# wenxiaoshuai/Points-Matching

Measured on AMD Instinct MI355X. Metric: descriptor-pair distances/s (BF-L2 2-NN + ratio stage); RANSAC hypotheses/s in `ransac`, higher is better.
Workload: dtype f32

## Files before the change

### include/pm.h

```cpp
#ifndef PM_H_
#define PM_H_

#include <stddef.h>
#include <stdint.h>

#ifdef __cplusplus
extern "C" {
#endif

#define PM_VERSION_MAJOR 0
#define PM_VERSION_MINOR 1

typedef enum pm_status {
    PM_OK            =  0,
    PM_E_INVALID     = -1,
    PM_E_TOO_FEW     = -2,
    PM_E_NO_MODEL    = -3,
    PM_E_HIP         = -4,
    PM_E_NOMEM       = -5,
    PM_E_UNSUPPORTED = -6
} pm_status;

typedef struct pm_match {
    int32_t queryIdx;
// ... 7 lines not shown
int  pm_ctx_create(int device, pm_ctx** out);
int  pm_ctx_destroy(pm_ctx* ctx);
int  pm_ctx_set_stream(pm_ctx* ctx, void* hip_stream);
int  pm_ctx_synchronize(pm_ctx* ctx);
int  pm_device_alloc(pm_ctx* ctx, size_t bytes, void** d_out);
int  pm_device_free(pm_ctx* ctx, void* d_ptr);
int  pm_device_upload(pm_ctx* ctx, void* d_dst, const void* src, size_t bytes);
int  pm_device_download(pm_ctx* ctx, void* dst, const void* d_src, size_t bytes);
int  pm_ctx_timing_enable(pm_ctx* ctx, int enable);
int  pm_ctx_timing_reset(pm_ctx* ctx);
int  pm_ctx_timing_get(pm_ctx* ctx, const char* kernel, double* mean_ms, int* launches);
int  pm_ctx_knn_diag_enable(pm_ctx* ctx, int enable);
int  pm_ctx_knn_stats(pm_ctx* ctx, int* rescans, int* nonfinite);
int  pm_ctx_knn_route(pm_ctx* ctx, int* route);
int  pm_ctx_filter_fusion_status(pm_ctx* ctx, int* gave_up);
enum {
    PM_OPT_RANSAC_PATH    = 1,
    PM_OPT_SCORE_OPERANDS = 2,
    PM_OPT_HAMMING_ROUTE  = 3,
    PM_OPT_KNN_F16_WAVES  = 4,
    PM_OPT_KNN_STAGING    = 6,
    PM_OPT_KNN_WG_PER_CU  = 7,
    PM_OPT_FILTER_FUSION  = 5,
    PM_OPT_KNN_XCD_TILE   = 8,
    PM_OPT_KNN_GENERAL_F16 = 9,
    PM_OPT_KNN_SEEDED     = 10,
    PM_OPT_KNN_U8_GROUP   = 11,
    PM_OPT_KNN_RING       = 12,
    PM_OPT_KNN_U8_REFINE  = 13,
    PM_OPT_KNN_RING_PROLOGUE = 14,
// ... 418 lines not shown
```

### points_matching_amd/api.py

```python
import ctypes as C
import os

import numpy as np

_HERE = os.path.dirname(os.path.abspath(__file__))
LIB_PATH = os.environ.get("PM_LIB_PATH") or os.path.join(_HERE, "libpm_hip.so")

MATCH_DTYPE = np.dtype([("queryIdx", "<i4"), ("trainIdx", "<i4"), ("imgIdx", "<i4"),
                        ("distance", "<f4")])
PM_MAX_K = 16
PM_KNN_FORCE_EXACT = 1
PM_KNN_FORCE_F32 = 2
PM_KNN_HINT_INTEGER = 4
PM_KNN_HINT_U8 = 8
PM_KNN_HINT_UNIT_NORM = 16
PM_CROSS_RATIO_FWD = 1
PM_CROSS_RATIO_REV = 2
PM_GUIDE_F_SAMPSON = 0
PM_GUIDE_F_SYM = 1
PM_GUIDE_H = 2
PM_ERR_SAMPSON = 0
PM_ERR_SYM_EPIPOLAR = 1
PM_ERR_REPROJ = 2
PM_AFFINE_FULL = 0
PM_AFFINE_PARTIAL = 1
PM_OK, PM_E_INVALID, PM_E_TOO_FEW, PM_E_NO_MODEL, PM_E_HIP, PM_E_NOMEM, PM_E_UNSUPPORTED = \
    0, -1, -2, -3, -4, -5, -6

EXPORTS = [
    "pm_ctx_create", "pm_ctx_destroy", "pm_ctx_set_stream", "pm_ctx_synchronize",
    "pm_ctx_timing_enable", "pm_ctx_timing_reset", "pm_ctx_timing_get", "pm_ctx_knn_diag_enable", "pm_ctx_knn_stats", "pm_ctx_knn_route",
    "pm_ctx_filter_fusion_status",
    "pm_last_error",
    "pm_status_string", "pm_version",
    "pm_bf_knn_l2_f32", "pm_bf_knn_l2_f32_dev", "pm_bf_knn_hamming_u8", "pm_bf_knn_hamming_u8_dev",
    "pm_filter_midpoint", "pm_filter_ratio", "pm_match_indices", "pm_gather_points",
    "pm_format_match_list",
    "pm_filter_ratio_gather_dev", "pm_filter_midpoint_gather_dev", "pm_concat_points_dev",
    "pm_ransac_fundamental", "pm_ransac_score_dev", "pm_ransac_score_devn", "pm_ransac_model_from_hyp",
    "pm_ransac_model_from_key_dev", "pm_ransac_run_dev", "pm_ransac_shard_parts_dev", "pm_ransac_finish_parts_dev",
    "pm_ctx_set_option", "pm_ctx_get_option", "pm_bf_knn_l2_ratio_dev",
    "pm_flann_build", "pm_flann_destroy", "pm_flann_knn_l2_f32", "pm_flann_knn_l2_f32_dev", "pm_flann_export",
    "pm_mgpu_create", "pm_mgpu_destroy", "pm_mgpu_size", "pm_mgpu_ctx", "pm_mgpu_ransac_fundamental", "pm_mgpu_match_ransac",
    "pm_mgpu_lane_ctx", "pm_mgpu_set_lanes", "pm_mgpu_set_train", "pm_mgpu_set_train_dev", "pm_mgpu_submit_dev", "pm_mgpu_collect",
    "pm_mgpu_allgather_latency", "pm_mgpu_batch_run", "pm_mgpu_batch_set_option",
    "pm_batch_create", "pm_batch_destroy", "pm_batch_run", "pm_batch_set_option", "pm_batch_set_desc_type", "pm_batch_set_host_threads",
    "pm_bf_knn_l2_u8", "pm_bf_knn_l2_u8_dev", "pm_bf_knn_l2_u8_ratio_dev", "pm_host_register", "pm_host_unregister",
# ... 331 lines not shown
    def ransac_finish_parts_dev(self, view, thresh_px, drecs_ptr, n_records, dkey_ptr, dF_ptr, dmask_ptr, mask_len,
                                dninl_ptr, dntotal_ptr=0, kind=PM_ERR_SAMPSON):
        prm = RansacParams(0, 0, 0, thresh_px, kind)
        _check(lib().pm_ransac_finish_parts_dev(self._h, C.byref(view), C.byref(prm), C.c_void_p(drecs_ptr), n_records,
                                                C.c_void_p(dkey_ptr or 0), C.c_void_p(dF_ptr or 0), C.c_void_p(dmask_ptr),
                                                mask_len, C.c_void_p(dninl_ptr or 0), C.c_void_p(dntotal_ptr or 0)))

    def knn_diag_enable(self, on=True):
        _check(lib().pm_ctx_knn_diag_enable(self._h, int(on)))

    def filter_fusion_gave_up(self):
        g = C.c_int()
        _check(lib().pm_ctx_filter_fusion_status(self._h, C.byref(g)))
        return g.value

    def knn_stats(self):
        r, nf = C.c_int(), C.c_int()
        _check(lib().pm_ctx_knn_stats(self._h, C.byref(r), C.byref(nf)))
        rt = C.c_int()
        _check(lib().pm_ctx_knn_route(self._h, C.byref(rt)))
        return {"rescans": r.value, "nonfinite": nf.value, "route": rt.value}

    def filter_ratio_gather_dev(self, dknn_ptr, nq, k, ratio, dkp1_ptr, dkp2_ptr, dgood_ptr, dxy1_ptr,
                                dxy2_ptr, dn_ptr):
        _check(lib().pm_filter_ratio_gather_dev(self._h, C.c_void_p(dknn_ptr), nq, k, C.c_float(ratio),
                                                C.c_void_p(dkp1_ptr), C.c_void_p(dkp2_ptr),
                                                C.c_void_p(dgood_ptr), C.c_void_p(dxy1_ptr),
                                                C.c_void_p(dxy2_ptr), C.c_void_p(dn_ptr)))

    def filter_cross_gather_dev(self, dfwd_ptr, nq, kf, drev_ptr, nt, kr, cross_flags, ratio, dkp1_ptr, dkp2_ptr, dgood_ptr,
# ... 936 lines not shown
```

### points_matching_amd/csrc/pm_capi.cpp

```cpp
#include <cfloat>
#include <cmath>

#include "pm_common.hpp"

namespace pm {

static thread_local char g_err[512] = "";

void set_error(const char* fmt, ...)
{
    va_list ap;
    va_start(ap, fmt);
    vsnprintf(g_err, sizeof g_err, fmt, ap);
    va_end(ap);
}

int arena_reserve(pm_ctx* ctx, size_t bytes)
{
    if (bytes <= ctx->arena_cap) return PM_OK;
    PM_HIP_CHECK(hipStreamSynchronize(ctx->stream));
    if (ctx->arena) PM_HIP_CHECK(hipFree(ctx->arena));
    ctx->arena = nullptr;
    ctx->arena_cap = 0;
    size_t cap = align_up(bytes + bytes / 4, size_t(1) << 20);
// ... 161 lines not shown
    *out = c;
    return PM_OK;
}

int pm_ctx_destroy(pm_ctx* ctx)
{
    if (!ctx) return PM_OK;
    (void)hipSetDevice(ctx->device);
    (void)hipStreamSynchronize(ctx->stream);
    drain_timers(ctx);
    for (hipEvent_t e : ctx->event_pool) (void)hipEventDestroy(e);
    if (ctx->arena) (void)hipFree(ctx->arena);
    if (ctx->knn_stats) (void)hipFree(ctx->knn_stats);
    if (ctx->fg_counts) (void)hipFree(ctx->fg_counts);
    if (ctx->sync_words) (void)hipFree(ctx->sync_words);
    if (ctx->kf_tile) (void)hipFree(ctx->kf_tile);
    if (ctx->widen) (void)hipFree(ctx->widen);
    if (ctx->feat) (void)hipFree(ctx->feat);
    if (ctx->pinned) (void)hipHostFree(ctx->pinned);
    if (ctx->own_stream) (void)hipStreamDestroy(ctx->own_stream);
    delete ctx;
    return PM_OK;
}

int pm_ctx_set_stream(pm_ctx* ctx, void* hip_stream)
{
    PM_REQUIRE(ctx != nullptr, PM_E_INVALID, "ctx is null");
    PM_HIP_CHECK(hipStreamSynchronize(ctx->stream));
    ctx->stream = hip_stream ? static_cast<hipStream_t>(hip_stream) : ctx->own_stream;
    return PM_OK;
// ... 102 lines not shown

int pm_ctx_knn_diag_enable(pm_ctx* ctx, int enable)
{
    PM_REQUIRE(ctx != nullptr, PM_E_INVALID, "ctx is null");
    ctx->knn_diag = enable != 0;
    return PM_OK;
}

int pm_ctx_filter_fusion_status(pm_ctx* ctx, int* gave_up)
{
    PM_REQUIRE(ctx != nullptr && gave_up != nullptr, PM_E_INVALID, "null argument");
    unsigned w = 0;
    PM_HIP_CHECK(hipStreamSynchronize(ctx->stream));
    PM_HIP_CHECK(hipMemcpy(&w, reinterpret_cast<const char*>(ctx->knn_stats) + 48, sizeof w, hipMemcpyDeviceToHost));
    *gave_up = (ctx->kf_epoch != 0u && w == ctx->kf_epoch) ? 1 : 0;
    return PM_OK;
}

int pm_ctx_knn_stats(pm_ctx* ctx, int* rescans, int* nonfinite)
{
    PM_REQUIRE(ctx != nullptr, PM_E_INVALID, "ctx is null");
    unsigned h[2] = {0, 0};
    PM_HIP_CHECK(hipStreamSynchronize(ctx->stream));
    PM_HIP_CHECK(hipMemcpy(h, ctx->knn_diag_words, sizeof h, hipMemcpyDeviceToHost));
    if (rescans) *rescans = static_cast<int>(h[0]);
    if (nonfinite) *nonfinite = static_cast<int>(h[1]);
    return PM_OK;
}

int pm_ctx_knn_route(pm_ctx* ctx, int* route)
// ... 206 lines not shown
```

### points_matching_amd/csrc/pm_common.hpp

```cpp
#pragma once
#include <hip/hip_runtime.h>

#include <cstdarg>
#include <cstdint>
#include <cstdio>
#include <cstring>
#include <map>
#include <string>
#include <vector>

#include "pm.h"
#include "stage_layout.hpp"

namespace pm {

void set_error(const char* fmt, ...);

#define PM_HIP_CHECK(expr)                                                              \
    do {                                                                                \
        hipError_t e_ = (expr);                                                         \
        if (e_ != hipSuccess) {                                                         \
            ::pm::set_error("%s failed: %s (%s:%d)", #expr, hipGetErrorString(e_),      \
                            __FILE__, __LINE__);                                        \
            return PM_E_HIP;                                                            \
// ... 38 lines not shown
    size_t pinned_cap = 0;
    bool timing = false;
    std::map<std::string, pm::KernelTimer> timers;
    std::vector<hipEvent_t> event_pool;
    int n_cu = 256;
    unsigned long long* knn_stats = nullptr;
    unsigned* knn_diag_words = nullptr;
    unsigned knn_epoch = 0;
    bool knn_diag = false;
    unsigned* fg_counts = nullptr;
    unsigned fg_epoch = 0;
    unsigned long long* kf_tile = nullptr;
    int kf_cap = 0;
    unsigned kf_epoch = 0;
    int* sync_words = nullptr;
    int opts[PM_OPT_COUNT_] = {};
    float* widen = nullptr;
    size_t widen_cap = 0;
    char* feat = nullptr;
    size_t feat_cap = 0;
    size_t feat_counter_off = 0;
    int feat_noct = 0;
    int feat_w[16] = {}, feat_h[16] = {};
    size_t feat_off[16] = {};
};

namespace pm {

int arena_reserve(pm_ctx* ctx, size_t bytes);
void arena_reset(pm_ctx* ctx);
// ... 83 lines not shown
```

### points_matching_amd/csrc/ransac_a_fused.hip

```cpp
#include "affine_core.hpp"
#include "ransac_fused_kernels.hpp"

namespace pm_ransac {
namespace {

using namespace pm_affine;

constexpr int RA_SYNC_WORD = 12;

template <int MODEL>
struct AModel {
    static constexpr int MIN_PTS = Traits<MODEL>::MIN_PTS;
    static constexpr bool SHARD_OUT = false;
    static constexpr int OUT_WORDS = 6;
    static constexpr bool CANDIDATES = false;

    template <typename DIAG>
    static __device__ __forceinline__ bool solve(const pm_points_view& v, const int* __restrict__ offs, int n, uint64_t seed,
                                                 uint64_t h, double (&A)[9])
    {
        int idx[MIN_PTS];
        sample<MODEL>(seed, h, n, idx);
        double x1[MIN_PTS], y1[MIN_PTS], x2[MIN_PTS], y2[MIN_PTS];
#pragma unroll
// ... 20 lines not shown
    }

    static __device__ __forceinline__ void inlier_x2(const float (&a)[9], f32x2 x, f32x2 y, f32x2 xp, f32x2 yp, float thr2,
                                                     bool& ia, bool& ib)
    {
        inlier_a32_x2(a, x, y, xp, yp, thr2, ia, ib);
    }
};

}

int ransac_a_enqueue(pm_ctx* ctx, int model, const pm_points_view& v, const pm_ransac_params* p, unsigned long long* d_key,
                     double* d_A, uint8_t* d_mask, int mask_len, int* d_ninl)
{
    if (model == PM_AFFINE_FULL)
        return fused_lds_enqueue<AModel<FULL>>(ctx, v, p, RA_SYNC_WORD, "ransac_a_fused", d_key, d_A, d_mask, mask_len, d_ninl);
    return fused_lds_enqueue<AModel<PARTIAL>>(ctx, v, p, RA_SYNC_WORD, "ransac_a_fused", d_key, d_A, d_mask, mask_len, d_ninl);
}

}
```

### points_matching_amd/csrc/ransac_e_fused.hip

```cpp
#include "ransac_fused_kernels.hpp"

namespace pm_ransac {
namespace {

constexpr int RE_SYNC_WORD = 16;

struct EModel {
    static constexpr int MIN_PTS = 5;
    static constexpr bool SHARD_OUT = false;
    static constexpr int OUT_WORDS = 9;
    static constexpr bool CANDIDATES = true;

    static __device__ __forceinline__ bool load(const double* __restrict__ cand, int k, double (&E)[9])
    {
        const double* c = cand + 10 * static_cast<size_t>(k);
#pragma unroll
        for (int i = 0; i < 9; ++i) E[i] = c[i];
        return c[9] != 0.0;
    }
    static __device__ __forceinline__ void inlier_pk(const ModelS& m, f32x2 x, f32x2 y, f32x2 xp, f32x2 yp, float thr2, bool& ia,
                                                     bool& ib)
    {
        FModel<PM_ERR_SAMPSON>::inlier_pk(m, x, y, xp, yp, thr2, ia, ib);
    }
    static __device__ __forceinline__ void inlier_x2(const float (&f)[9], f32x2 x, f32x2 y, f32x2 xp, f32x2 yp, float thr2,
                                                     bool& ia, bool& ib)
    {
        FModel<PM_ERR_SAMPSON>::inlier_x2(f, x, y, xp, yp, thr2, ia, ib);
    }
};

}

int ransac_e_enqueue(pm_ctx* ctx, const pm_points_view& vn, const pm_ransac_params* q, const double* d_cand,
                     unsigned long long* d_key, double* d_E, uint8_t* d_mask, int mask_len, int* d_ninl)
{
    return fused_lds_enqueue<EModel>(ctx, vn, q, RE_SYNC_WORD, "ransac_e_fused", d_key, d_E, d_mask, mask_len, d_ninl, d_cand);
}

}
```

### points_matching_amd/csrc/ransac_fused_kernels.hpp

```cpp
#pragma once
#include <type_traits>

#include "ransac_core.hpp"
#include "ransac_internal.hpp"

namespace pm_ransac {
namespace {

constexpr int RF_THREADS = 256;
constexpr int RF_TEAMS = 2;
constexpr int RF_WG = RF_THREADS * RF_TEAMS;
constexpr int RF_PTS_PER_SLOT = 2 * RF_THREADS;
constexpr int RF_PPT2 = 5;
constexpr int RF_PPT2_BIG = 10;
static_assert(RF_PPT2_BIG <= 10, "score_tile is instantiated for 1..10 slots");

struct RfSlot {
    unsigned long long key;
    double F[9];
    unsigned long long pad[6];
};
static_assert(sizeof(RfSlot) == 128, "slot stride");

struct RfOut {
// ... 388 lines not shown
    }
    const int covered = n > 0 ? (n + RF_PTS_PER_SLOT - 1) / RF_PTS_PER_SLOT * RF_PTS_PER_SLOT : 0;
    for (int i = covered + tid; i < out.mask_len; i += RF_WG) out.mask[i] = 0;
    __syncthreads();
    if (tid == 0) {
        int tot = 0;
#pragma unroll
        for (int w = 0; w < RF_THREADS / 64; ++w) tot += s_wc[w];
        if (out.n_inliers) *out.n_inliers = tot;
        if (out.fo) out.fo->n_inliers = tot;
    }
    DIAG::phase(8);
    DIAG::phase(9);
}

constexpr int RL_WAVES = 12;
constexpr int RL_THREADS = RL_WAVES * 64;
constexpr int RL_SLOT_PTS = 128;
constexpr int RL_MAX_SLOTS = 64;

struct GeomF {
    static constexpr bool OWN = false;
    static constexpr int PLANES = 4, MW = 12, FLAG = 9, WORDS = 9, MAX_SLOTS = RL_MAX_SLOTS;
};
template <typename M, typename = void>
struct GeomOf {
    using type = GeomF;
};
template <typename M>
struct GeomOf<M, std::void_t<typename M::Geom>> {
// ... 73 lines not shown
            for (int h = 0; h < NH; ++h) {
                bool ia, ib;
                MODEL::inlier_pk(ms[h], x, y, xp, yp, thr2, ia, ib);
                c[h] += __popcll(__ballot(ia)) + __popcll(__ballot(ib));
            }
        }
        if (lane == 0) {
#pragma unroll
            for (int h = 0; h < NH; ++h) s_cnt[ss[h]] += c[h];
        }
    }
}

template <typename MODEL, typename DIAG>
__global__ __launch_bounds__(RL_THREADS) void ransac_fused_lds(pm_points_view v, uint64_t seed, int64_t hyp_begin, int nh, int hb,
                                                               float thr2, int tile_slots, RfSlot* __restrict__ slots,
                                                               int* __restrict__ ticket, RfOut out)
{
    using G = typename GeomOf<MODEL>::type;
    extern __shared__ __attribute__((aligned(16))) f32x2 s_pts[];
    __shared__ __attribute__((aligned(16))) float s_mdl[RF_HB_MAX][G::MW];
    __shared__ double s_m64[RF_HB_MAX][G::WORDS];
    __shared__ int s_cnt[RF_HB_MAX];
    __shared__ int s_offs[PM_MAX_PARTS + 1];
    __shared__ unsigned long long s_wk[RL_WAVES];
    __shared__ double s_F64[G::WORDS];
    __shared__ int s_role;
    __shared__ int s_wc[RL_WAVES];

    const int tid = threadIdx.x, lane = tid & 63, wave = tid >> 6;
    DIAG::phase(0);
    int n;
    if (v.parts == 1) {
        n = view_count1(v);
    } else {
        view_offsets(v, s_offs, tid);
        __syncthreads();
        n = s_offs[v.parts];
    }
    DIAG::phase(1);
    const int tile_pts = tile_slots * RL_SLOT_PTS;
    const int ntiles = n > tile_pts ? (n + tile_pts - 1) / tile_pts : 1;
    const float nanv = __builtin_nanf("");
    auto load_pair = [&](int base, int slot, int l) {
        const int i0 = base + 2 * (64 * slot + l);
        if constexpr (G::OWN) {
// ... 91 lines not shown
                else if (k == 3) score_lds_ids<MODEL, 3, G>(s_mdl, s_cnt, s_pts + lane, kslots, ss, thr2, lane);
                else if (k == 2) score_lds_ids<MODEL, 2, G>(s_mdl, s_cnt, s_pts + lane, kslots, ss, thr2, lane);
                else score_lds_ids<MODEL, 1, G>(s_mdl, s_cnt, s_pts + lane, kslots, ss, thr2, lane);
            }
        } else {
            for (int s = wave; s < hcount; s += 4 * RL_WAVES) {
                const int left = (hcount - s + RL_WAVES - 1) / RL_WAVES;
                if (left >= 4) score_lds<MODEL, 4>(s_mdl, s_cnt, s_pts + lane, kslots, s, thr2, lane);
                else if (left == 3) score_lds<MODEL, 3>(s_mdl, s_cnt, s_pts + lane, kslots, s, thr2, lane);
                else if (left == 2) score_lds<MODEL, 2>(s_mdl, s_cnt, s_pts + lane, kslots, s, thr2, lane);
                else score_lds<MODEL, 1>(s_mdl, s_cnt, s_pts + lane, kslots, s, thr2, lane);
            }
        }
    }
    DIAG::phase(5);
    __syncthreads();

    unsigned long long key = 0ull;
    if (tid < hcount && s_mdl[tid][G::FLAG] != 0.f)
        key = (static_cast<unsigned long long>(static_cast<uint32_t>(s_cnt[tid])) << 32) |
              static_cast<unsigned long long>(0xFFFFFFFFu - static_cast<uint32_t>(hyp_begin + h0 + tid));
    const unsigned long long kbest = wg_max_u64<RL_WAVES>(key, s_wk, tid);
    if (wave == 0) {
        const int sb = kbest ? static_cast<int>(static_cast<int64_t>(0xFFFFFFFFu - static_cast<uint32_t>(kbest)) - hyp_begin) - h0 : 0;
        double* sf = reinterpret_cast<double*>(slots) + static_cast<size_t>(lane) * gridDim.x + blockIdx.x;
        if (lane < G::WORDS) __hip_atomic_store(sf, kbest ? s_m64[sb][lane] : 0.0, __ATOMIC_RELAXED, __HIP_MEMORY_SCOPE_AGENT);
        if (lane == G::WORDS) __hip_atomic_store(reinterpret_cast<unsigned long long*>(sf), kbest, __ATOMIC_RELAXED, __HIP_MEMORY_SCOPE_AGENT);
        asm volatile("s_waitcnt vmcnt(0)" ::: "memory");
        if (lane == 0) {
            const int tk = __hip_atomic_fetch_add(ticket, 1, __ATOMIC_RELAXED, __HIP_MEMORY_SCOPE_AGENT);
            s_role = tk == static_cast<int>(gridDim.x) - 1 ? 1 : 0;
        }
    }
    __syncthreads();
    DIAG::phase(6);
    if (s_role == 0) { DIAG::phase(9); return; }

    if (tid == 0) __hip_atomic_store(ticket, 0, __ATOMIC_RELAXED, __HIP_MEMORY_SCOPE_AGENT);
    unsigned long long kb = 0ull;
    double fb[G::WORDS];
#pragma unroll
    for (int i = 0; i < G::WORDS; ++i) fb[i] = 0.0;
    for (int j = tid; j < static_cast<int>(gridDim.x); j += RL_THREADS) {
        const double* sf = reinterpret_cast<const double*>(slots) + j;
        const unsigned long long kj = __hip_atomic_load(reinterpret_cast<const unsigned long long*>(sf + G::WORDS * static_cast<size_t>(gridDim.x)),
                                                        __ATOMIC_RELAXED, __HIP_MEMORY_SCOPE_AGENT);
        double fj[G::WORDS];
#pragma unroll
        for (int i = 0; i < G::WORDS; ++i) fj[i] = __hip_atomic_load(sf + i * static_cast<size_t>(gridDim.x), __ATOMIC_RELAXED, __HIP_MEMORY_SCOPE_AGENT);
        if (kj > kb) {
            kb = kj;
#pragma unroll
            for (int i = 0; i < G::WORDS; ++i) fb[i] = fj[i];
        }
    }
    const unsigned long long kwin = wg_max_u64<RL_WAVES>(kb, s_wk, tid);
    const bool ok = kwin != 0ull && n >= MODEL::MIN_PTS;
    if (tid < G::WORDS) s_F64[tid] = 0.0;
    __syncthreads();
    if (ok && kb == kwin) {
#pragma unroll
        for (int i = 0; i < G::WORDS; ++i) s_F64[i] = fb[i];
    }
    __syncthreads();
    DIAG::phase(7);
    if (MODEL::SHARD_OUT && out.shard) {
        if (tid < 9) out.rec->F[tid] = s_F64[tid];
        if (tid == 9) out.rec->key = ok ? kwin : 0ull;
        return;
    }
    if (tid < G::WORDS) {
        if (out.F && (MODEL::OUT_WORDS == G::WORDS || tid < MODEL::OUT_WORDS)) out.F[tid] = s_F64[tid];
        if (MODEL::SHARD_OUT && out.fo) { out.fo->F[tid] = s_F64[tid]; out.fo->F32[tid] = static_cast<float>(s_F64[tid]); }
    }
    if (tid == G::WORDS) {
        *out.key = ok ? kwin : 0ull;
        if (MODEL::SHARD_OUT && out.fo) out.fo->valid = ok ? 1 : 0;
    }
    float fw[G::OWN ? G::MW : 9];
    if constexpr (G::OWN) {
        MODEL::mask_model(out.cand, ok, kwin, hyp_begin, fw);
    } else {
#pragma unroll
        for (int i = 0; i < 9; ++i) fw[i] = static_cast<float>(s_F64[i]);
    }
    int mine = 0;
    for (int t = 0; t < ntiles; ++t) {
        const int kslots = tile_kslots(t);
        if (ntiles > 1) {
            __syncthreads();
            for (int slot = wave; slot < kslots; slot += RL_WAVES) load_pair(t * tile_pts, slot, lane);
            __syncthreads();
        }
        for (int slot = wave; slot < kslots; slot += RL_WAVES) {
            const f32x2* pp = s_pts + static_cast<size_t>(slot) * (64 * G::PLANES) + lane;
            bool ia, ib;
            if constexpr (G::OWN) {
                f32x2 op[G::PLANES];
#pragma unroll
                for (int q = 0; q < G::PLANES; ++q) op[q] = pp[64 * q];
                MODEL::inlier_x2(fw, op, thr2, ia, ib);
            } else {
                MODEL::inlier_x2(fw, pp[0], pp[64], pp[128], pp[192], thr2, ia, ib);
            }
            ia = ia && ok; ib = ib && ok;
            const int i0 = t * tile_pts + 2 * (64 * slot + lane);
            if (i0 < out.mask_len) out.mask[i0] = ia ? 1 : 0;
            if (i0 + 1 < out.mask_len) out.mask[i0 + 1] = ib ? 1 : 0;
            mine += __popcll(__ballot(ia)) + __popcll(__ballot(ib));
        }
    }
    if (lane == 0) s_wc[wave] = mine;
    const int covered = n > 0 ? (n + RL_SLOT_PTS - 1) / RL_SLOT_PTS * RL_SLOT_PTS : 0;
    for (int i = covered + tid; i < out.mask_len; i += RL_THREADS) out.mask[i] = 0;
    __syncthreads();
    if (tid == 0) {
        int tot = 0;
#pragma unroll
        for (int w = 0; w < RL_WAVES; ++w) tot += s_wc[w];
        if (out.n_inliers) *out.n_inliers = tot;
        if (MODEL::SHARD_OUT && out.fo) out.fo->n_inliers = tot;
    }
    DIAG::phase(8);
    DIAG::phase(9);
}

int sync_words(pm_ctx* ctx, int** out)
{
    if (!ctx->sync_words) {
        PM_HIP_CHECK(hipMalloc(reinterpret_cast<void**>(&ctx->sync_words), 256));
        PM_HIP_CHECK(hipMemsetAsync(ctx->sync_words, 0, 256, ctx->stream));
    }
    *out = ctx->sync_words;
    return PM_OK;
}

template <typename MODEL, typename DIAG>
int fused_lds_launch(pm_ctx* ctx, const pm_points_view& v, const pm_ransac_params* p, int nwg, int hb, RfSlot* slots,
                     int* ticket, const RfOut& out)
{
    using G = typename GeomOf<MODEL>::type;
    const long long cap_total = static_cast<long long>(v.parts) * v.cap;
    const long long need = (cap_total + RL_SLOT_PTS - 1) / RL_SLOT_PTS;
    const int tile_slots = static_cast<int>(need < 1 ? 1 : (need > G::MAX_SLOTS ? G::MAX_SLOTS : need));
    const size_t lds = static_cast<size_t>(tile_slots) * G::PLANES * 64 * sizeof(f32x2);
    static bool attr_done_dev[PM_MAX_DEVICES] = {};
    if (!attr_done_dev[ctx->device]) {
        PM_HIP_CHECK(hipFuncSetAttribute(reinterpret_cast<const void*>(&ransac_fused_lds<MODEL, DIAG>),
                                         hipFuncAttributeMaxDynamicSharedMemorySize,
                                         G::MAX_SLOTS * G::PLANES * 64 * static_cast<int>(sizeof(f32x2))));
        attr_done_dev[ctx->device] = true;
    }
    const float thr2 = p->thresh_px * p->thresh_px;
    hipLaunchKernelGGL((ransac_fused_lds<MODEL, DIAG>), dim3(nwg), dim3(RL_THREADS), lds, ctx->stream, v, p->seed, p->hyp_begin,
                       static_cast<int>(p->hyp_end - p->hyp_begin), hb, thr2, tile_slots, slots, ticket, out);
    PM_HIP_CHECK(hipGetLastError());
    return PM_OK;
}

template <typename MODEL>
int fused_lds_enqueue(pm_ctx* ctx, const pm_points_view& v, const pm_ransac_params* p, int sync_word, const char* timer,
                      unsigned long long* d_key, double* d_model, uint8_t* d_mask, int mask_len, int* d_ninl,
                      const double* d_cand = nullptr)
{
    const long long nh = p->hyp_end - p->hyp_begin;
    const int hb = fused_hb(ctx, nh);
    const int nwg = static_cast<int>((nh + hb - 1) / hb);
    RfSlot* slots = static_cast<RfSlot*>(pm::arena_take(ctx, sizeof(RfSlot) * static_cast<size_t>(nwg)));
    PM_REQUIRE(slots, PM_E_NOMEM, "scratch arena too small");
    int* sync = nullptr;
    int rc = sync_words(ctx, &sync);
    if (rc != PM_OK) return rc;
    RfOut out{};
    out.key = d_key; out.F = d_model; out.mask = d_mask; out.mask_len = mask_len; out.n_inliers = d_ninl;
    out.cand = d_cand;
    pm::ScopedKernelTime t(ctx, timer);
    return fused_lds_launch<MODEL, NoDiag>(ctx, v, p, nwg, hb, slots, sync + sync_word, out);
}

template <typename DIAG>
int fused_launch_t(pm_ctx* ctx, const pm_points_view& v, const pm_ransac_params* p, int shard, pm_ransac_record* d_rec,
                 unsigned long long* d_key, double* d_F, uint8_t* d_mask, int mask_len, int* d_ninl, FinalOut** fo_out)
{
    const long long nh = p->hyp_end - p->hyp_begin;
    const long long cap_total = static_cast<long long>(v.parts) * v.cap;
    PM_REQUIRE(nh >= 1, PM_E_INVALID, "fused_launch: empty hypothesis range");
    PM_REQUIRE(nh <= 0x7FFFFFFFLL, PM_E_INVALID, "a single launch takes at most 2^31 - 1 hypothesis ids: split the range");
    const int hb = fused_hb(ctx, nh);
    const int nwg = static_cast<int>((nh + hb - 1) / hb);
    RfSlot* slots = static_cast<RfSlot*>(pm::arena_take(ctx, sizeof(RfSlot) * static_cast<size_t>(nwg)));
    FinalOut* fo = static_cast<FinalOut*>(pm::arena_take(ctx, sizeof(FinalOut)));
    PM_REQUIRE(slots && fo, PM_E_NOMEM, "scratch arena too small");
    int* sync = nullptr;
    int rc = sync_words(ctx, &sync);
    if (rc != PM_OK) return rc;
    RfOut out{};
    out.shard = shard;
    out.key = d_key; out.F = d_F; out.mask = d_mask; out.mask_len = mask_len; out.n_inliers = d_ninl;
    out.fo = fo_out ? fo : nullptr;
    out.rec = d_rec;
    if (fo_out) *fo_out = fo;
    const float thr2 = p->thresh_px * p->thresh_px;
    pm::ScopedKernelTime t(ctx, "ransac_fused");
    if (ctx->opts[PM_OPT_RANSAC_FORM] != 1) {
        if (p->error_kind == PM_ERR_SAMPSON) return fused_lds_launch<FModel<PM_ERR_SAMPSON>, DIAG>(ctx, v, p, nwg, hb, slots, sync, out);
        return fused_lds_launch<FModel<PM_ERR_SYM_EPIPOLAR>, DIAG>(ctx, v, p, nwg, hb, slots, sync, out);
    }
#define PM_RF(KIND_, PPT2_)                                                                                              \
    hipLaunchKernelGGL((ransac_fused<KIND_, PPT2_, DIAG>), dim3(nwg), dim3(RF_WG), 0, ctx->stream, v, p->seed, p->hyp_begin, \
                       static_cast<int>(nh), hb, thr2, slots, sync, out)
    const int depth = cap_total <= 2 * RF_PTS_PER_SLOT ? 2 : (cap_total <= RF_PPT2 * RF_PTS_PER_SLOT ? RF_PPT2 : RF_PPT2_BIG);
#define PM_RF_K(KIND_)                                                                   \
    do {                                                                                 \
        if (depth == 2) PM_RF(KIND_, 2);                                                 \
        else if (depth == RF_PPT2) PM_RF(KIND_, RF_PPT2);                                \
        else PM_RF(KIND_, RF_PPT2_BIG);                                                  \
    } while (0)
    if (p->error_kind == PM_ERR_SAMPSON) PM_RF_K(PM_ERR_SAMPSON);
    else PM_RF_K(PM_ERR_SYM_EPIPOLAR);
#undef PM_RF_K
#undef PM_RF
    PM_HIP_CHECK(hipGetLastError());
// ... 6 lines not shown
```

### points_matching_amd/csrc/ransac_h_fused.hip

```cpp
#include "homography_core.hpp"
#include "ransac_fused_kernels.hpp"

namespace pm_ransac {
namespace {

using namespace pm_homog;

constexpr int RH_SYNC_WORD = 8;

struct HModel {
    static constexpr int MIN_PTS = 4;
    static constexpr bool SHARD_OUT = false;
    static constexpr int OUT_WORDS = 9;
    static constexpr bool CANDIDATES = false;

    template <typename DIAG>
    static __device__ __forceinline__ bool solve(const pm_points_view& v, const int* __restrict__ offs, int n, uint64_t seed,
                                                 uint64_t h, double (&H)[9])
    {
        int idx[4];
        sample4(seed, h, n, idx);
        double x1[4], y1[4], x2[4], y2[4];
#pragma unroll
        for (int i = 0; i < 4; ++i) {
// ... 19 lines not shown
        ib = (lhs[1] <= rhs[1]) && __builtin_amdgcn_classf(rhs[1], CLASS_POS_FINITE);
    }

    static __device__ __forceinline__ void inlier_x2(const float (&h)[9], f32x2 x, f32x2 y, f32x2 xp, f32x2 yp, float thr2,
                                                     bool& ia, bool& ib)
    {
        inlier_h32_x2(h, x, y, xp, yp, thr2, ia, ib);
    }
};

}

int ransac_h_enqueue(pm_ctx* ctx, const pm_points_view& v, const pm_ransac_params* p, unsigned long long* d_key,
                     double* d_H, uint8_t* d_mask, int mask_len, int* d_ninl)
{
    return fused_lds_enqueue<HModel>(ctx, v, p, RH_SYNC_WORD, "ransac_h_fused", d_key, d_H, d_mask, mask_len, d_ninl);
}

}
```

### points_matching_amd/csrc/ransac_p_fused.hip

```cpp
#include "pnp_core.hpp"
#include "ransac_fused_kernels.hpp"

namespace pm_ransac {
namespace {

using pm_pnp::SLOT_DOUBLES;

constexpr int RP_SYNC_WORD = 20;

struct PnpGeom {
    static constexpr bool OWN = true;
    static constexpr int PLANES = 5, MW = 16, FLAG = 12, WORDS = 12, MAX_SLOTS = 48;
};

__device__ __forceinline__ bool inlier1(const float (&P)[16], float x, float y, float z, float u, float v, float thr2)
{
    const float a = fmaf(P[0], x, fmaf(P[1], y, fmaf(P[2], z, P[3])));
    const float b = fmaf(P[4], x, fmaf(P[5], y, fmaf(P[6], z, P[7])));
    const float w = fmaf(P[8], x, fmaf(P[9], y, fmaf(P[10], z, P[11])));
    const float du = fmaf(-u, w, a), dv = fmaf(-v, w, b);
    const float lhs = fmaf(du, du, dv * dv), rhs = thr2 * (w * w);
    return lhs <= rhs && w > 0.0f && rhs > 0.0f && rhs < __builtin_inff();
}

// ... 67 lines not shown
        ib = lhs[1] <= rhs[1] && w[1] > 0.0f && rhs[1] > 0.0f && rhs[1] < __builtin_inff();
    }

    static __device__ __forceinline__ void inlier_x2(const float (&f)[16], const f32x2 (&op)[5], float thr2, bool& ia, bool& ib)
    {
        ia = inlier1(f, op[0][0], op[1][0], op[2][0], op[3][0], op[4][0], thr2);
        ib = inlier1(f, op[0][1], op[1][1], op[2][1], op[3][1], op[4][1], thr2);
    }
};

}

int ransac_p_enqueue(pm_ctx* ctx, const pm_points_view& v, const pm_ransac_params* q, const double* d_cand,
                     unsigned long long* d_key, double* d_Rt, uint8_t* d_mask, int mask_len, int* d_ninl)
{
    return fused_lds_enqueue<PModel>(ctx, v, q, RP_SYNC_WORD, "ransac_p_fused", d_key, d_Rt, d_mask, mask_len, d_ninl, d_cand);
}

}
```

### points_matching_amd/csrc/ransac_shard.hip

```cpp
#include "ransac_fused_kernels.hpp"

namespace pm_ransac {
namespace {

template <int KIND>
__global__ __launch_bounds__(RF_THREADS) void ransac_finish(pm_points_view v, const pm_ransac_record* __restrict__ recs, int nrec,
                                                            float thr2, unsigned long long* __restrict__ key_out,
                                                            double* __restrict__ F_out, uint8_t* __restrict__ mask, int mask_len,
                                                            int* __restrict__ n_inl_out, int* __restrict__ n_total_out,
                                                            int* __restrict__ sync)
{
    __shared__ int s_offs[PM_MAX_PARTS + 1];
    __shared__ unsigned long long s_wk[RF_THREADS / 64];
    __shared__ int s_wc[RF_THREADS / 64];
    __shared__ int s_last;
    const int tid = threadIdx.x, lane = tid & 63, wave = tid >> 6;
    if (v.parts > 1) view_offsets(v, s_offs, tid);
    unsigned long long kb = 0ull;
    for (int j = tid; j < nrec; j += RF_THREADS) { const unsigned long long kj = recs[j].key; kb = kj > kb ? kj : kb; }
    const unsigned long long kwin = wg_max_u64<RF_THREADS / 64>(kb, s_wk, tid);
    const int n = v.parts > 1 ? s_offs[v.parts] : view_count1(v);
    const bool ok = kwin != 0ull && n >= 8;
    int owner = 0;
    for (int j = 0; j < nrec; ++j) owner = recs[j].key == kwin ? j : owner;
// ... 45 lines not shown
        return ctx->opts[PM_OPT_RANSAC_WG_IDS] < RF_HB_MAX ? ctx->opts[PM_OPT_RANSAC_WG_IDS] : RF_HB_MAX;
    const long long wgs = ctx->n_cu;
    const long long per_round = wgs * RF_HB_MAX;
    const long long rounds = (nh + per_round - 1) / per_round;
    long long hb = (nh + wgs * rounds - 1) / (wgs * rounds);
    if (hb < 1) hb = 1;
    if (hb > RF_HB_MAX) hb = RF_HB_MAX;
    return static_cast<int>(hb);
}

size_t fused_scratch_bytes(const pm_ctx* ctx, const pm_ransac_params* p)
{
    const long long nh = p->hyp_end - p->hyp_begin;
    const int hb = fused_hb(ctx, nh);
    const long long nwg = (nh + hb - 1) / hb;
    return pm::align_up(sizeof(RfSlot) * static_cast<size_t>(nwg > 0 ? nwg : 1), 256) + pm::align_up(sizeof(FinalOut), 256) + 512;
}

}

using namespace pm_ransac;


extern "C" int pm_ransac_shard_parts_dev(pm_ctx* ctx, const pm_points_view* view, const pm_ransac_params* p,
                                         pm_ransac_record* d_record)
{
    PM_REQUIRE(ctx != nullptr && d_record != nullptr && p != nullptr, PM_E_INVALID, "null argument");
    int rc = check_view(view);
    if (rc != PM_OK) return rc;
    PM_REQUIRE(p->hyp_begin >= 0 && p->hyp_end > p->hyp_begin && p->hyp_end <= 0x100000000LL, PM_E_INVALID,
               "hypothesis ids must satisfy 0 <= begin < end <= 2^32");
// ... 36 lines not shown
```

Measured before the change: 2320 billion.

## Replace last-block ticket reduction with epoch-tagged spin-wait tail in fused RANSAC

The fused LDS RANSAC kernel no longer has every workgroup publish its best model and bump an atomic ticket so that whichever finishes last does the final reduction. Now each producer block writes epoch-tagged 32-bit halves of its key and model into a persistent per-context tail buffer, and the fixed last block spin-waits on those tags, with a timeout that reports a give-up status. This removes the ticket atomic and the extra barrier from every block, plus the arena slot allocation. The cost is a reliance on the last block being scheduled alongside the producers, and a timeout path. Inlier mask bytes are also written in pairs as 16-bit stores.

After: 2261 billion. 2.5% lower.

```diff
diff --git a/include/pm.h b/include/pm.h
--- a/include/pm.h
+++ b/include/pm.h
@@ -45,6 +45,7 @@
 int  pm_ctx_knn_stats(pm_ctx* ctx, int* rescans, int* nonfinite);
 int  pm_ctx_knn_route(pm_ctx* ctx, int* route);
 int  pm_ctx_filter_fusion_status(pm_ctx* ctx, int* gave_up);
+int  pm_ctx_ransac_tail_status(pm_ctx* ctx, int* gave_up);
 enum {
     PM_OPT_RANSAC_PATH    = 1,
     PM_OPT_SCORE_OPERANDS = 2,
diff --git a/points_matching_amd/api.py b/points_matching_amd/api.py
--- a/points_matching_amd/api.py
+++ b/points_matching_amd/api.py
@@ -30,7 +30,7 @@
 EXPORTS = [
     "pm_ctx_create", "pm_ctx_destroy", "pm_ctx_set_stream", "pm_ctx_synchronize",
     "pm_ctx_timing_enable", "pm_ctx_timing_reset", "pm_ctx_timing_get", "pm_ctx_knn_diag_enable", "pm_ctx_knn_stats", "pm_ctx_knn_route",
-    "pm_ctx_filter_fusion_status",
+    "pm_ctx_filter_fusion_status", "pm_ctx_ransac_tail_status",
     "pm_last_error",
     "pm_status_string", "pm_version",
     "pm_bf_knn_l2_f32", "pm_bf_knn_l2_f32_dev", "pm_bf_knn_hamming_u8", "pm_bf_knn_hamming_u8_dev",
@@ -392,6 +392,11 @@
         _check(lib().pm_ctx_filter_fusion_status(self._h, C.byref(g)))
         return g.value
 
+    def ransac_tail_gave_up(self):
+        g = C.c_int()
+        _check(lib().pm_ctx_ransac_tail_status(self._h, C.byref(g)))
+        return g.value
+
     def knn_stats(self):
         r, nf = C.c_int(), C.c_int()
         _check(lib().pm_ctx_knn_stats(self._h, C.byref(r), C.byref(nf)))
diff --git a/points_matching_amd/csrc/pm_capi.cpp b/points_matching_amd/csrc/pm_capi.cpp
--- a/points_matching_amd/csrc/pm_capi.cpp
+++ b/points_matching_amd/csrc/pm_capi.cpp
@@ -199,6 +199,7 @@
     if (ctx->knn_stats) (void)hipFree(ctx->knn_stats);
     if (ctx->fg_counts) (void)hipFree(ctx->fg_counts);
     if (ctx->sync_words) (void)hipFree(ctx->sync_words);
+    if (ctx->rt_block) (void)hipFree(ctx->rt_block);
     if (ctx->kf_tile) (void)hipFree(ctx->kf_tile);
     if (ctx->widen) (void)hipFree(ctx->widen);
     if (ctx->feat) (void)hipFree(ctx->feat);
@@ -331,6 +332,19 @@
     PM_HIP_CHECK(hipStreamSynchronize(ctx->stream));
     PM_HIP_CHECK(hipMemcpy(&w, reinterpret_cast<const char*>(ctx->knn_stats) + 48, sizeof w, hipMemcpyDeviceToHost));
     *gave_up = (ctx->kf_epoch != 0u && w == ctx->kf_epoch) ? 1 : 0;
+    return PM_OK;
+}
+
+int pm_ctx_ransac_tail_status(pm_ctx* ctx, int* gave_up)
+{
+    PM_REQUIRE(ctx != nullptr && gave_up != nullptr, PM_E_INVALID, "null argument");
+    *gave_up = 0;
+    if (!ctx->rt_block) return PM_OK;
+    unsigned long long h[17] = {};
+    PM_HIP_CHECK(hipStreamSynchronize(ctx->stream));
+    PM_HIP_CHECK(hipMemcpy(h, ctx->rt_block, sizeof h, hipMemcpyDeviceToHost));
+    const unsigned epoch = static_cast<unsigned>(h[0]), status = static_cast<unsigned>(h[16]);
+    *gave_up = (status != 0u && status == epoch) ? 1 : 0;
     return PM_OK;
 }
 
diff --git a/points_matching_amd/csrc/pm_common.hpp b/points_matching_amd/csrc/pm_common.hpp
--- a/points_matching_amd/csrc/pm_common.hpp
+++ b/points_matching_amd/csrc/pm_common.hpp
@@ -76,6 +76,8 @@
     int kf_cap = 0;
     unsigned kf_epoch = 0;
     int* sync_words = nullptr;
+    unsigned long long* rt_block = nullptr;
+    int rt_cap = 0;
     int opts[PM_OPT_COUNT_] = {};
     float* widen = nullptr;
     size_t widen_cap = 0;
diff --git a/points_matching_amd/csrc/ransac_a_fused.hip b/points_matching_amd/csrc/ransac_a_fused.hip
--- a/points_matching_amd/csrc/ransac_a_fused.hip
+++ b/points_matching_amd/csrc/ransac_a_fused.hip
@@ -6,7 +6,6 @@
 
 using namespace pm_affine;
 
-constexpr int RA_SYNC_WORD = 12;
 
 template <int MODEL>
 struct AModel {
@@ -58,8 +57,8 @@
                      double* d_A, uint8_t* d_mask, int mask_len, int* d_ninl)
 {
     if (model == PM_AFFINE_FULL)
-        return fused_lds_enqueue<AModel<FULL>>(ctx, v, p, RA_SYNC_WORD, "ransac_a_fused", d_key, d_A, d_mask, mask_len, d_ninl);
-    return fused_lds_enqueue<AModel<PARTIAL>>(ctx, v, p, RA_SYNC_WORD, "ransac_a_fused", d_key, d_A, d_mask, mask_len, d_ninl);
+        return fused_lds_enqueue<AModel<FULL>>(ctx, v, p, "ransac_a_fused", d_key, d_A, d_mask, mask_len, d_ninl);
+    return fused_lds_enqueue<AModel<PARTIAL>>(ctx, v, p, "ransac_a_fused", d_key, d_A, d_mask, mask_len, d_ninl);
 }
 
 }
diff --git a/points_matching_amd/csrc/ransac_e_fused.hip b/points_matching_amd/csrc/ransac_e_fused.hip
--- a/points_matching_amd/csrc/ransac_e_fused.hip
+++ b/points_matching_amd/csrc/ransac_e_fused.hip
@@ -3,7 +3,6 @@
 namespace pm_ransac {
 namespace {
 
-constexpr int RE_SYNC_WORD = 16;
 
 struct EModel {
     static constexpr int MIN_PTS = 5;
@@ -35,7 +34,7 @@
 int ransac_e_enqueue(pm_ctx* ctx, const pm_points_view& vn, const pm_ransac_params* q, const double* d_cand,
                      unsigned long long* d_key, double* d_E, uint8_t* d_mask, int mask_len, int* d_ninl)
 {
-    return fused_lds_enqueue<EModel>(ctx, vn, q, RE_SYNC_WORD, "ransac_e_fused", d_key, d_E, d_mask, mask_len, d_ninl, d_cand);
+    return fused_lds_enqueue<EModel>(ctx, vn, q, "ransac_e_fused", d_key, d_E, d_mask, mask_len, d_ninl, d_cand);
 }
 
 }
diff --git a/points_matching_amd/csrc/ransac_fused_kernels.hpp b/points_matching_amd/csrc/ransac_fused_kernels.hpp
--- a/points_matching_amd/csrc/ransac_fused_kernels.hpp
+++ b/points_matching_amd/csrc/ransac_fused_kernels.hpp
@@ -426,6 +426,12 @@
     DIAG::phase(9);
 }
 
+typedef __attribute__((address_space(1))) unsigned long long gu64;
+typedef __attribute__((address_space(1))) unsigned gu32;
+constexpr int RT_EPOCH_WORD = 0, RT_STATUS_WORD = 16, RT_HDR_WORDS = 32;
+constexpr int RT_NG_MAX = 26;
+constexpr unsigned long long RT_SPIN_TICKS = 200000000ull;
+
 constexpr int RL_WAVES = 12;
 constexpr int RL_THREADS = RL_WAVES * 64;
 constexpr int RL_SLOT_PTS = 128;
@@ -529,10 +535,12 @@
 
 template <typename MODEL, typename DIAG>
 __global__ __launch_bounds__(RL_THREADS) void ransac_fused_lds(pm_points_view v, uint64_t seed, int64_t hyp_begin, int nh, int hb,
-                                                               float thr2, int tile_slots, RfSlot* __restrict__ slots,
-                                                               int* __restrict__ ticket, RfOut out)
+                                                               float thr2, int tile_slots, unsigned long long* tail, int cap_wg,
+                                                               RfOut out)
 {
     using G = typename GeomOf<MODEL>::type;
+    constexpr int NG = 2 * (G::WORDS + 1);
+    static_assert(NG <= RT_NG_MAX && NG <= 64, "one lane of wave 0 per granule; the block holds RT_NG_MAX arrays");
     extern __shared__ __attribute__((aligned(16))) f32x2 s_pts[];
     __shared__ __attribute__((aligned(16))) float s_mdl[RF_HB_MAX][G::MW];
     __shared__ double s_m64[RF_HB_MAX][G::WORDS];
@@ -540,11 +548,16 @@
     __shared__ int s_offs[PM_MAX_PARTS + 1];
     __shared__ unsigned long long s_wk[RL_WAVES];
     __shared__ double s_F64[G::WORDS];
-    __shared__ int s_role;
+    __shared__ int s_gave_up;
     __shared__ int s_wc[RL_WAVES];
 
     const int tid = threadIdx.x, lane = tid & 63, wave = tid >> 6;
     DIAG::phase(0);
+    gu32* const g_epoch = (gu32*)(tail + RT_EPOCH_WORD);
+    gu32* const g_status = (gu32*)(tail + RT_STATUS_WORD);
+    gu64* const gran = (gu64*)(tail + RT_HDR_WORDS);
+    unsigned tag = __hip_atomic_load(g_epoch, __ATOMIC_RELAXED, __HIP_MEMORY_SCOPE_AGENT) + 1u;
+    tag = static_cast<unsigned>(__builtin_amdgcn_readfirstlane(static_cast<int>(tag ? tag : 1u)));
     int n;
     if (v.parts == 1) {
         n = view_count1(v);
@@ -666,6 +679,7 @@
         }
     }
     DIAG::phase(5);
+    if (tid == 0) s_gave_up = 0;
     __syncthreads();
 
     unsigned long long key = 0ull;
@@ -673,42 +687,64 @@
         key = (static_cast<unsigned long long>(static_cast<uint32_t>(s_cnt[tid])) << 32) |
               static_cast<unsigned long long>(0xFFFFFFFFu - static_cast<uint32_t>(hyp_begin + h0 + tid));
     const unsigned long long kbest = wg_max_u64<RL_WAVES>(key, s_wk, tid);
-    if (wave == 0) {
-        const int sb = kbest ? static_cast<int>(static_cast<int64_t>(0xFFFFFFFFu - static_cast<uint32_t>(kbest)) - hyp_begin) - h0 : 0;
-        double* sf = reinterpret_cast<double*>(slots) + static_cast<size_t>(lane) * gridDim.x + blockIdx.x;
-        if (lane < G::WORDS) __hip_atomic_store(sf, kbest ? s_m64[sb][lane] : 0.0, __ATOMIC_RELAXED, __HIP_MEMORY_SCOPE_AGENT);
-        if (lane == G::WORDS) __hip_atomic_store(reinterpret_cast<unsigned long long*>(sf), kbest, __ATOMIC_RELAXED, __HIP_MEMORY_SCOPE_AGENT);
-        asm volatile("s_waitcnt vmcnt(0)" ::: "memory");
-        if (lane == 0) {
-            const int tk = __hip_atomic_fetch_add(ticket, 1, __ATOMIC_RELAXED, __HIP_MEMORY_SCOPE_AGENT);
-            s_role = tk == static_cast<int>(gridDim.x) - 1 ? 1 : 0;
-        }
-    }
-    __syncthreads();
+    const int sb = kbest ? static_cast<int>(static_cast<int64_t>(0xFFFFFFFFu - static_cast<uint32_t>(kbest)) - hyp_begin) - h0 : 0;
+    const int nprod = static_cast<int>(gridDim.x) - 1;
+    if (static_cast<int>(blockIdx.x) != nprod) {
+        if (wave == 0 && lane < NG) {
+            const int w = lane >> 1;
+            unsigned long long x = kbest;
+            if (w < G::WORDS) x = kbest ? static_cast<unsigned long long>(__double_as_longlong(s_m64[sb][w])) : 0ull;
+            const unsigned half = static_cast<unsigned>(x >> (32 * (lane & 1)));
+            __hip_atomic_store(gran + static_cast<size_t>(lane) * cap_wg + blockIdx.x,
+                               (static_cast<unsigned long long>(tag) << 32) | half, __ATOMIC_RELAXED, __HIP_MEMORY_SCOPE_AGENT);
+        }
+        DIAG::phase(6);
+        DIAG::phase(9);
+        return;
+    }
     DIAG::phase(6);
-    if (s_role == 0) { DIAG::phase(9); return; }
-
-    if (tid == 0) __hip_atomic_store(ticket, 0, __ATOMIC_RELAXED, __HIP_MEMORY_SCOPE_AGENT);
+
     unsigned long long kb = 0ull;
     double fb[G::WORDS];
 #pragma unroll
     for (int i = 0; i < G::WORDS; ++i) fb[i] = 0.0;
-    for (int j = tid; j < static_cast<int>(gridDim.x); j += RL_THREADS) {
-        const double* sf = reinterpret_cast<const double*>(slots) + j;
-        const unsigned long long kj = __hip_atomic_load(reinterpret_cast<const unsigned long long*>(sf + G::WORDS * static_cast<size_t>(gridDim.x)),
-                                                        __ATOMIC_RELAXED, __HIP_MEMORY_SCOPE_AGENT);
-        double fj[G::WORDS];
-#pragma unroll
-        for (int i = 0; i < G::WORDS; ++i) fj[i] = __hip_atomic_load(sf + i * static_cast<size_t>(gridDim.x), __ATOMIC_RELAXED, __HIP_MEMORY_SCOPE_AGENT);
-        if (kj > kb) {
+    for (int j0 = wave * 64; j0 < nprod; j0 += RL_THREADS) {
+        const int j = j0 + lane;
+        const bool act = j < nprod;
+        const gu64* g = gran + (act ? j : j0);
+        unsigned val[NG];
+        const unsigned long long t0 = __builtin_amdgcn_s_memrealtime();
+        bool seen;
+        for (;;) {
+            bool ok = true;
+#pragma unroll
+            for (int k = 0; k < NG; ++k) {
+                const unsigned long long x = __hip_atomic_load(g + static_cast<size_t>(k) * cap_wg, __ATOMIC_RELAXED, __HIP_MEMORY_SCOPE_AGENT);
+                val[k] = static_cast<unsigned>(x);
+                ok = ok && static_cast<unsigned>(x >> 32) == tag;
+            }
+            seen = __all(ok || !act);
+            if (seen || __builtin_amdgcn_s_memrealtime() - t0 > RT_SPIN_TICKS) break;
+            __builtin_amdgcn_s_sleep(4);
+        }
+        if (!seen) {
+            if (lane == 0) s_gave_up = 1;
+            break;
+        }
+        const unsigned long long kj = (static_cast<unsigned long long>(val[2 * G::WORDS + 1]) << 32) | val[2 * G::WORDS];
+        if (act && kj > kb) {
             kb = kj;
 #pragma unroll
-            for (int i = 0; i < G::WORDS; ++i) fb[i] = fj[i];
-        }
-    }
-    const unsigned long long kwin = wg_max_u64<RL_WAVES>(kb, s_wk, tid);
-    const bool ok = kwin != 0ull && n >= MODEL::MIN_PTS;
-    if (tid < G::WORDS) s_F64[tid] = 0.0;
+            for (int i = 0; i < G::WORDS; ++i)
+                fb[i] = __longlong_as_double(static_cast<long long>((static_cast<unsigned long long>(val[2 * i + 1]) << 32) | val[2 * i]));
+        }
+    }
+    const unsigned long long kswept = wg_max_u64<RL_WAVES>(kb, s_wk, tid);
+    const bool gave_up = s_gave_up != 0;
+    const unsigned long long kwin = kswept > kbest ? kswept : kbest;
+    const bool ok = !gave_up && kwin != 0ull && n >= MODEL::MIN_PTS;
+    if (gave_up && tid == 0) __hip_atomic_store(g_status, tag, __ATOMIC_RELAXED, __HIP_MEMORY_SCOPE_AGENT);
+    if (tid < G::WORDS) s_F64[tid] = ok && kwin == kbest ? s_m64[sb][tid] : 0.0;
     __syncthreads();
     if (ok && kb == kwin) {
 #pragma unroll
@@ -719,6 +755,7 @@
     if (MODEL::SHARD_OUT && out.shard) {
         if (tid < 9) out.rec->F[tid] = s_F64[tid];
         if (tid == 9) out.rec->key = ok ? kwin : 0ull;
+        if (tid == 0) __hip_atomic_store(g_epoch, tag, __ATOMIC_RELAXED, __HIP_MEMORY_SCOPE_AGENT);
         return;
     }
     if (tid < G::WORDS) {
@@ -737,6 +774,7 @@
         for (int i = 0; i < 9; ++i) fw[i] = static_cast<float>(s_F64[i]);
     }
     int mine = 0;
+    const bool pair16 = (reinterpret_cast<uintptr_t>(out.mask) & 1u) == 0;
     for (int t = 0; t < ntiles; ++t) {
         const int kslots = tile_kslots(t);
         if (ntiles > 1) {
@@ -757,8 +795,12 @@
             }
             ia = ia && ok; ib = ib && ok;
             const int i0 = t * tile_pts + 2 * (64 * slot + lane);
-            if (i0 < out.mask_len) out.mask[i0] = ia ? 1 : 0;
-            if (i0 + 1 < out.mask_len) out.mask[i0 + 1] = ib ? 1 : 0;
+            if (pair16 && i0 + 1 < out.mask_len) {
+                *reinterpret_cast<uint16_t*>(out.mask + i0) = static_cast<uint16_t>((ia ? 1u : 0u) | (ib ? 0x100u : 0u));
+            } else {
+                if (i0 < out.mask_len) out.mask[i0] = ia ? 1 : 0;
+                if (i0 + 1 < out.mask_len) out.mask[i0 + 1] = ib ? 1 : 0;
+            }
             mine += __popcll(__ballot(ia)) + __popcll(__ballot(ib));
         }
     }
@@ -772,6 +814,7 @@
         for (int w = 0; w < RL_WAVES; ++w) tot += s_wc[w];
         if (out.n_inliers) *out.n_inliers = tot;
         if (MODEL::SHARD_OUT && out.fo) out.fo->n_inliers = tot;
+        __hip_atomic_store(g_epoch, tag, __ATOMIC_RELAXED, __HIP_MEMORY_SCOPE_AGENT);
     }
     DIAG::phase(8);
     DIAG::phase(9);
@@ -787,11 +830,32 @@
     return PM_OK;
 }
 
+int tail_block(pm_ctx* ctx, int nwg, unsigned long long** out)
+{
+    if (nwg > ctx->rt_cap) {
+        PM_REQUIRE(!pm::stream_is_capturing(ctx->stream), PM_E_UNSUPPORTED,
+                   "the stream is capturing a graph and the RANSAC tail block must grow: make one call of this size before the capture");
+        PM_HIP_CHECK(hipStreamSynchronize(ctx->stream));
+        if (ctx->rt_block) PM_HIP_CHECK(hipFree(ctx->rt_block));
+        ctx->rt_block = nullptr;
+        ctx->rt_cap = 0;
+        const int cap = nwg < 1024 ? 1024 : nwg + nwg / 2;
+        const size_t bytes = 8 * (RT_HDR_WORDS + static_cast<size_t>(RT_NG_MAX) * cap);
+        PM_HIP_CHECK(hipMalloc(reinterpret_cast<void**>(&ctx->rt_block), bytes));
+        PM_HIP_CHECK(hipMemsetAsync(ctx->rt_block, 0, bytes, ctx->stream));
+        ctx->rt_cap = cap;
+    }
+    *out = ctx->rt_block;
+    return PM_OK;
+}
+
 template <typename MODEL, typename DIAG>
-int fused_lds_launch(pm_ctx* ctx, const pm_points_view& v, const pm_ransac_params* p, int nwg, int hb, RfSlot* slots,
-                     int* ticket, const RfOut& out)
+int fused_lds_launch(pm_ctx* ctx, const pm_points_view& v, const pm_ransac_params* p, int nwg, int hb, const RfOut& out)
 {
     using G = typename GeomOf<MODEL>::type;
+    unsigned long long* tail = nullptr;
+    const int rc = tail_block(ctx, nwg, &tail);
+    if (rc != PM_OK) return rc;
     const long long cap_total = static_cast<long long>(v.parts) * v.cap;
     const long long need = (cap_total + RL_SLOT_PTS - 1) / RL_SLOT_PTS;
     const int tile_slots = static_cast<int>(need < 1 ? 1 : (need > G::MAX_SLOTS ? G::MAX_SLOTS : need));
@@ -805,29 +869,24 @@
     }
     const float thr2 = p->thresh_px * p->thresh_px;
     hipLaunchKernelGGL((ransac_fused_lds<MODEL, DIAG>), dim3(nwg), dim3(RL_THREADS), lds, ctx->stream, v, p->seed, p->hyp_begin,
-                       static_cast<int>(p->hyp_end - p->hyp_begin), hb, thr2, tile_slots, slots, ticket, out);
+                       static_cast<int>(p->hyp_end - p->hyp_begin), hb, thr2, tile_slots, tail, ctx->rt_cap, out);
     PM_HIP_CHECK(hipGetLastError());
     return PM_OK;
 }
 
 template <typename MODEL>
-int fused_lds_enqueue(pm_ctx* ctx, const pm_points_view& v, const pm_ransac_params* p, int sync_word, const char* timer,
+int fused_lds_enqueue(pm_ctx* ctx, const pm_points_view& v, const pm_ransac_params* p, const char* timer,
                       unsigned long long* d_key, double* d_model, uint8_t* d_mask, int mask_len, int* d_ninl,
                       const double* d_cand = nullptr)
 {
     const long long nh = p->hyp_end - p->hyp_begin;
     const int hb = fused_hb(ctx, nh);
     const int nwg = static_cast<int>((nh + hb - 1) / hb);
-    RfSlot* slots = static_cast<RfSlot*>(pm::arena_take(ctx, sizeof(RfSlot) * static_cast<size_t>(nwg)));
-    PM_REQUIRE(slots, PM_E_NOMEM, "scratch arena too small");
-    int* sync = nullptr;
-    int rc = sync_words(ctx, &sync);
-    if (rc != PM_OK) return rc;
     RfOut out{};
     out.key = d_key; out.F = d_model; out.mask = d_mask; out.mask_len = mask_len; out.n_inliers = d_ninl;
     out.cand = d_cand;
     pm::ScopedKernelTime t(ctx, timer);
-    return fused_lds_launch<MODEL, NoDiag>(ctx, v, p, nwg, hb, slots, sync + sync_word, out);
+    return fused_lds_launch<MODEL, NoDiag>(ctx, v, p, nwg, hb, out);
 }
 
 template <typename DIAG>
@@ -840,12 +899,10 @@
     PM_REQUIRE(nh <= 0x7FFFFFFFLL, PM_E_INVALID, "a single launch takes at most 2^31 - 1 hypothesis ids: split the range");
     const int hb = fused_hb(ctx, nh);
     const int nwg = static_cast<int>((nh + hb - 1) / hb);
-    RfSlot* slots = static_cast<RfSlot*>(pm::arena_take(ctx, sizeof(RfSlot) * static_cast<size_t>(nwg)));
+    const bool lds_form = ctx->opts[PM_OPT_RANSAC_FORM] != 1;
+    RfSlot* slots = lds_form ? nullptr : static_cast<RfSlot*>(pm::arena_take(ctx, sizeof(RfSlot) * static_cast<size_t>(nwg)));
     FinalOut* fo = static_cast<FinalOut*>(pm::arena_take(ctx, sizeof(FinalOut)));
-    PM_REQUIRE(slots && fo, PM_E_NOMEM, "scratch arena too small");
-    int* sync = nullptr;
-    int rc = sync_words(ctx, &sync);
-    if (rc != PM_OK) return rc;
+    PM_REQUIRE((lds_form || slots) && fo, PM_E_NOMEM, "scratch arena too small");
     RfOut out{};
     out.shard = shard;
     out.key = d_key; out.F = d_F; out.mask = d_mask; out.mask_len = mask_len; out.n_inliers = d_ninl;
@@ -854,10 +911,13 @@
     if (fo_out) *fo_out = fo;
     const float thr2 = p->thresh_px * p->thresh_px;
     pm::ScopedKernelTime t(ctx, "ransac_fused");
-    if (ctx->opts[PM_OPT_RANSAC_FORM] != 1) {
-        if (p->error_kind == PM_ERR_SAMPSON) return fused_lds_launch<FModel<PM_ERR_SAMPSON>, DIAG>(ctx, v, p, nwg, hb, slots, sync, out);
-        return fused_lds_launch<FModel<PM_ERR_SYM_EPIPOLAR>, DIAG>(ctx, v, p, nwg, hb, slots, sync, out);
-    }
+    if (lds_form) {
+        if (p->error_kind == PM_ERR_SAMPSON) return fused_lds_launch<FModel<PM_ERR_SAMPSON>, DIAG>(ctx, v, p, nwg, hb, out);
+        return fused_lds_launch<FModel<PM_ERR_SYM_EPIPOLAR>, DIAG>(ctx, v, p, nwg, hb, out);
+    }
+    int* sync = nullptr;
+    const int rc = sync_words(ctx, &sync);
+    if (rc != PM_OK) return rc;
 #define PM_RF(KIND_, PPT2_)                                                                                              \
     hipLaunchKernelGGL((ransac_fused<KIND_, PPT2_, DIAG>), dim3(nwg), dim3(RF_WG), 0, ctx->stream, v, p->seed, p->hyp_begin, \
                        static_cast<int>(nh), hb, thr2, slots, sync, out)
diff --git a/points_matching_amd/csrc/ransac_h_fused.hip b/points_matching_amd/csrc/ransac_h_fused.hip
--- a/points_matching_amd/csrc/ransac_h_fused.hip
+++ b/points_matching_amd/csrc/ransac_h_fused.hip
@@ -6,7 +6,6 @@
 
 using namespace pm_homog;
 
-constexpr int RH_SYNC_WORD = 8;
 
 struct HModel {
     static constexpr int MIN_PTS = 4;
@@ -57,7 +56,7 @@
 int ransac_h_enqueue(pm_ctx* ctx, const pm_points_view& v, const pm_ransac_params* p, unsigned long long* d_key,
                      double* d_H, uint8_t* d_mask, int mask_len, int* d_ninl)
 {
-    return fused_lds_enqueue<HModel>(ctx, v, p, RH_SYNC_WORD, "ransac_h_fused", d_key, d_H, d_mask, mask_len, d_ninl);
+    return fused_lds_enqueue<HModel>(ctx, v, p, "ransac_h_fused", d_key, d_H, d_mask, mask_len, d_ninl);
 }
 
 }
diff --git a/points_matching_amd/csrc/ransac_p_fused.hip b/points_matching_amd/csrc/ransac_p_fused.hip
--- a/points_matching_amd/csrc/ransac_p_fused.hip
+++ b/points_matching_amd/csrc/ransac_p_fused.hip
@@ -6,7 +6,6 @@
 
 using pm_pnp::SLOT_DOUBLES;
 
-constexpr int RP_SYNC_WORD = 20;
 
 struct PnpGeom {
     static constexpr bool OWN = true;
@@ -105,7 +104,7 @@
 int ransac_p_enqueue(pm_ctx* ctx, const pm_points_view& v, const pm_ransac_params* q, const double* d_cand,
                      unsigned long long* d_key, double* d_Rt, uint8_t* d_mask, int mask_len, int* d_ninl)
 {
-    return fused_lds_enqueue<PModel>(ctx, v, q, RP_SYNC_WORD, "ransac_p_fused", d_key, d_Rt, d_mask, mask_len, d_ninl, d_cand);
+    return fused_lds_enqueue<PModel>(ctx, v, q, "ransac_p_fused", d_key, d_Rt, d_mask, mask_len, d_ninl, d_cand);
 }
 
 }
diff --git a/points_matching_amd/csrc/ransac_shard.hip b/points_matching_amd/csrc/ransac_shard.hip
--- a/points_matching_amd/csrc/ransac_shard.hip
+++ b/points_matching_amd/csrc/ransac_shard.hip
@@ -83,7 +83,8 @@
     const long long nh = p->hyp_end - p->hyp_begin;
     const int hb = fused_hb(ctx, nh);
     const long long nwg = (nh + hb - 1) / hb;
-    return pm::align_up(sizeof(RfSlot) * static_cast<size_t>(nwg > 0 ? nwg : 1), 256) + pm::align_up(sizeof(FinalOut), 256) + 512;
+    const size_t slots = ctx->opts[PM_OPT_RANSAC_FORM] == 1 ? pm::align_up(sizeof(RfSlot) * static_cast<size_t>(nwg > 0 ? nwg : 1), 256) : 0;
+    return slots + pm::align_up(sizeof(FinalOut), 256) + 512;
 }
 
 }
```
